# cgtuebingen/ggnn

Hardware: AMD Instinct MI355X
Metric: queries/sec @ recall@10 (SIFT1M-shaped, k=10) (higher is better)
Workload: dtype f32

## Files before the change

ggnn_amd/_lib.py:

```python
import ctypes as C
import os

_HERE = os.path.dirname(os.path.abspath(__file__))
LIB_PATH = os.path.join(_HERE, "csrc", "libggnn_amd.so")
if os.environ.get("GGNN_TEST_HOOKS") == "1" and os.environ.get("GGNN_AMD_LIB"):
    LIB_PATH = os.environ["GGNN_AMD_LIB"]

OK, INVALID_ARGUMENT, INVALID_STATE, OUT_OF_RANGE, OUT_OF_MEMORY, DEVICE_ERROR, UNSUPPORTED, \
    IO_ERROR = range(8)
F32, U8, F16, BF16 = 0, 1, 2, 3
I8 = 5
CPU, GPU = 0, 1


class GraphConfig(C.Structure):
    _fields_ = [(n, C.c_uint32) for n in
                ("N", "D", "KBuild", "KF", "G", "S", "S0", "S0_off", "SG", "SG_off", "N_all",
                 "ST_all")] + [("Bs", C.c_uint32 * 4), ("Ns", C.c_uint32 * 4),
                               ("Ns_offsets", C.c_uint32 * 4), ("STs_offsets", C.c_uint32 * 4)]

    def as_dict(self):
        d = {}
        for name, _ in self._fields_:
            v = getattr(self, name)
# ... 125 lines not shown
    "ggnn_last_build_work": (_int, [_vp, C.POINTER(BuildWork)]),
    "ggnn_last_query_parts": (_int, [_vp, C.POINTER(_u32)]),
    "ggnn_rccl_ranks": (_int, [_vp, C.POINTER(_u32)]),
    "ggnn_set_hook": (_int, [C.c_char_p, C.c_int64]),
    "ggnn_reset_hook": (_int, [C.c_char_p]),
    "ggnn_get_hook": (_int, [C.c_char_p, C.POINTER(C.c_int64)]),
    "ggnn_set_log_level": (None, [_int]),
    "ggnn_graph_config_init": (_int, [_u32, _u32, _u32, _cfgp]),
    "ggnn_query_sizing": (_int, [_u32, _u32, _u32, C.POINTER(_u32), C.POINTER(_u32)]),
    "ggnn_op_dist_layout": (_int, [_u32, _int, C.POINTER(_u32), C.POINTER(_u32)]),
    "ggnn_op_query": (_int, [_vp, _int, _u32, _u32, _vp, _u32, _vp, _u32, _vp, _u32, _vp, _u32,
                             _f32, _u32, _int, _u32, _u32, _vp, _vp, _vp, _vp, _vp]),
    "ggnn_prescreen_sizes": (_int, [_u32, _u32, _int, C.POINTER(_u32), C.POINTER(_sz),
                                    C.POINTER(_sz)]),
    "ggnn_op_prescreen_encode": (_int, [_vp, _u32, _u32, _int, _vp, _vp, _vp, _vp]),
    "ggnn_op_prescreen_probe": (_int, [_vp, _vp, _u32, _int, _vp, _u32, _vp, _u32, _vp, _vp, _vp,
                                       _vp]),
    "ggnn_op_query_prescreened": (_int, [_vp, _u32, _u32, _vp, _vp, _vp, _u32, _vp, _u32, _vp, _u32,
                                         _vp, _u32, _f32, _u32, _int, _u32, _u32, _vp, _vp, _vp,
                                         _vp, _vp, _vp]),
    "ggnn_op_query_filtered": (_int, [_vp, _int, _u32, _u32, _vp, _vp, _vp, _u32, _vp, _u32, _vp,
                                      _u32, _vp, _u32, _f32, _u32, _int, _u32, _u32, _vp, _vp, _vp,
                                      _vp, _vp, _vp, _u32, _vp]),
    "ggnn_op_bf_query_filtered": (_int, [_vp, _int, _u32, _u32, _vp, _u32, _u32, _int, _vp, _vp,
                                         _vp, _u32, _vp]),
    "ggnn_op_query_filtered_by": (_int, [_vp, _int, _u32, _u32, _vp, _vp, _vp, _u32, _vp, _u32,
                                         _vp, _u32, _vp, _u32, _f32, _u32, _int, _u32, _u32, _vp,
                                         _vp, _vp, _vp, _vp, _vp, _u32, _u64, _vp, _u32, _vp]),
    "ggnn_op_bf_query_filtered_by": (_int, [_vp, _int, _u32, _u32, _vp, _u32, _u32, _int, _vp,
                                            _vp, _vp, _u32, _u64, _vp, _u32, _vp]),
# ... 140 lines not shown
```

ggnn_amd/csrc/common.hpp:

```cpp
#pragma once
#include <hip/hip_runtime.h>

#include <cstdint>
#include <cstdio>
#include <stdexcept>
#include <string>

#include "../../include/ggnn_c.h"

namespace ggnn_amd {

constexpr int kWave = 64;
constexpr int32_t kEmptyKey = -1;
constexpr uint32_t kLayers = 4;
constexpr uint32_t kKBlock = 32;

struct Error : std::runtime_error {
  ggnn_status status;
  Error(ggnn_status s, const std::string& msg) : std::runtime_error(msg), status(s) {}
};

#define GGNN_HIP_CHECK(expr)                                                                  \
  do {                                                                                        \
    hipError_t _e = (expr);                                                                   \
// ... 121 lines not shown
  uint32_t num_start;
  const float* nn1_stats;
  uint32_t k_query;
  float tau_query;
  uint32_t max_iterations;
  ggnn_measure measure;
  uint32_t shards_per_gpu, on_gpu_shard;
  int32_t* ids;
  float* dists;
  uint32_t* n_dist;
  uint32_t* n_pop;
  const uint8_t* ps_codes{nullptr};
  const float* ps_params{nullptr};
  uint32_t ps_Dc{0};
  bool ps_lossless{false};
  uint32_t* n_rows{nullptr};
  const uint32_t* filter_bits{nullptr};
  uint32_t filter_bit_offset{0};
  FilterTable filter_table{};
  LabelSetSpec label_sets{};
  LabelRangeSpec label_ranges{};
  LabelMaskSpec label_masks{};
};
void launch_query(const QueryLaunch& a, hipStream_t stream);

constexpr int kPsHeaderFloats = 8;
inline uint32_t prescreen_code_dim(uint32_t D)
{
  if (D <= 64) {
    uint32_t p = 16;
    while (p < D)
      p <<= 1;
    return p;
  }
  return (D + 63u) / 64u * 64u;
}
size_t prescreen_param_floats(uint32_t D);
size_t prescreen_scratch_floats(uint32_t N, uint32_t D, ggnn_measure measure);
void launch_prescreen_encode(const float* base, uint32_t N, uint32_t D, ggnn_measure measure,
                             uint8_t* codes, float* params, float* scratch, hipStream_t stream);
void launch_prescreen_probe(const uint8_t* codes, const float* params, uint32_t D,
                            ggnn_measure measure, const float* query, uint32_t Nq,
                            const int32_t* cand, uint32_t M, const float* crit, int32_t* reject,
                            float* s_out, hipStream_t stream);

struct BfLaunch {
  const void* base;
  const void* query;
  ggnn_dtype dtype;
  uint32_t N_base, D, Nq, k_query;
  ggnn_measure measure;
  int32_t* ids;
  float* dists;
  uint32_t* n_rescanned{nullptr};
  const uint32_t* filter_bits{nullptr};
// ... 180 lines not shown
```

ggnn_amd/csrc/engine.hpp:

```cpp
#pragma once
#include <dlfcn.h>
#include <rccl/rccl.h>

#include <algorithm>
#include <atomic>
#include <cstdlib>
#include <cstring>
#include <filesystem>
#include <fstream>
#include <exception>
#include <memory>
#include <mutex>
#include <thread>
#include <vector>

#include "common.hpp"
#include "hooks.hpp"

namespace ggnn_amd {

struct DeviceBuffer {
  void* p{nullptr};
  size_t bytes{0};
  DeviceBuffer() = default;
// ... 93 lines not shown
    GGNN_HIP_CHECK(hipEventSynchronize(b));
    GGNN_HIP_CHECK(hipEventElapsedTime(&ms, a, b));
    return ms;
  }
};

struct Shard {
  uint32_t global_id{0};
  DeviceBuffer pool;
  int32_t* graph{nullptr};
  int32_t* translation{nullptr};
  int32_t* selection{nullptr};
  float* nn1_stats{nullptr};
  bool ready{false};
  DeviceBuffer ps_codes, ps_params;
  int ps_state{0};
  bool ps_lossless{false};
  ggnn_measure ps_measure{GGNN_EUCLIDEAN};

  static size_t pool_bytes(const ggnn_graph_config& c)
  {
    return (static_cast<size_t>(c.N_all) * c.KBuild + 2 * static_cast<size_t>(c.ST_all)) * 4 +
           2 * sizeof(float);
  }
  void view(const ggnn_graph_config& c, void* slot_pool)
  {
    graph = static_cast<int32_t*>(slot_pool);
    translation = graph + static_cast<size_t>(c.N_all) * c.KBuild;
    selection = translation + c.ST_all;
    nn1_stats = reinterpret_cast<float*>(selection + c.ST_all);
// ... 517 lines not shown
```

ggnn_amd/csrc/engine_cabi.cpp:

```cpp
#include "engine.hpp"
#include "traversal.hpp"

namespace {
thread_local std::string g_create_error;

template <typename F>
ggnn_status guarded(ggnn_t* h, F&& f)
{
  DeviceRestoreGuard restore;
  try {
    f();
    return GGNN_OK;
  }
  catch (const Error& e) {
    (h ? h->last_error : g_create_error) = e.what();
    return e.status;
  }
  catch (const std::bad_alloc&) {
    (h ? h->last_error : g_create_error) = "out of host memory";
    return GGNN_OUT_OF_MEMORY;
  }
  catch (const std::exception& e) {
    (h ? h->last_error : g_create_error) = e.what();
    return GGNN_DEVICE_ERROR;
// ... 984 lines not shown
    if (scratch_floats)
      *scratch_floats = prescreen_scratch_floats(N_base, D, measure);
  });
}

ggnn_status ggnn_op_prescreen_encode(const float* base, uint32_t N_base, uint32_t D,
                                     ggnn_measure measure, uint8_t* codes, float* params,
                                     float* scratch, void* stream)
{
  return guarded(nullptr, [&] {
    launch_prescreen_encode(base, N_base, D, measure, codes, params, scratch,
                            static_cast<hipStream_t>(stream));
  });
}

ggnn_status ggnn_op_prescreen_probe(const uint8_t* codes, const float* params, uint32_t D,
                                    ggnn_measure measure, const float* query, uint32_t Nq,
                                    const int32_t* cand, uint32_t M, const float* crit,
                                    int32_t* reject, float* s_out, void* stream)
{
  return guarded(nullptr, [&] {
    launch_prescreen_probe(codes, params, D, measure, query, Nq, cand, M, crit, reject, s_out,
                           static_cast<hipStream_t>(stream));
  });
}

ggnn_status ggnn_op_query_prescreened(const float* base, uint32_t N_base, uint32_t D,
                                      const uint8_t* codes, const float* params,
                                      const float* query, uint32_t Nq, const int32_t* graph0,
                                      uint32_t KBuild, const int32_t* start, uint32_t num_start,
// ... 666 lines not shown
```

ggnn_amd/csrc/engine_query.cpp:

```cpp
#include "engine.hpp"

void ggnn_handle::check_query(uint64_t Nq, uint32_t D, ggnn_dtype dtype, const void* q) const
{
  GGNN_REQUIRE(dtype == base_dtype, GGNN_INVALID_ARGUMENT,
               "query data type does not match base data type");
  GGNN_REQUIRE(D == base_D, GGNN_INVALID_ARGUMENT, "query dimension does not match the base");
  GGNN_REQUIRE(Nq < 0xffffffffull, GGNN_INVALID_ARGUMENT, "too many queries");
  GGNN_REQUIRE(!Nq || q != nullptr, GGNN_INVALID_ARGUMENT, "query pointer is null");
}

ggnn_handle::Staged ggnn_handle::stage_query(DeviceCtx& ctx, const void* q, uint64_t Nq, uint32_t D, ggnn_dtype dtype,
                   ggnn_location loc, int q_gpu)
{
  Staged s;
  if (!Nq)
    return s;
  const size_t es = dtype_size(dtype);
  const bool padded = pad_D != base_D;
  if (loc == GGNN_GPU && q_gpu == ctx.device && !padded &&
      (reinterpret_cast<uintptr_t>(q) & 15u) == 0) {
    s.ptr = q;
    return s;
  }
  const hipMemcpyKind kind = loc == GGNN_GPU ? hipMemcpyDefault : hipMemcpyHostToDevice;
// ... 29 lines not shown
                 r.k,
                 r.tau,
                 r.max_iterations,
                 r.measure,
                 shards_per_gpu,
                 si,
                 d_ids,
                 d_dists,
                 nullptr,
                 nullptr};
  if (use_prescreen) {
    ql.ps_codes = sh.ps_codes.as<uint8_t>();
    ql.ps_params = sh.ps_params.as<float>();
    ql.ps_Dc = prescreen_code_dim(pad_D);
    ql.ps_lossless = sh.ps_lossless;
  }
  ql.filter_bits = df.bits;
  ql.filter_bit_offset = sh.global_id * cfg.N;
  ql.filter_table = df.table;
  ql.label_sets = df.set;
  ql.label_ranges = df.ranges;
  ql.label_masks = df.masks;
  return ql;
}

void ggnn_handle::query_device(DeviceCtx& ctx, const QueryRequest& r, const void* d_query,
                               int32_t* d_ids, float* d_dists, const QueryFilter& filter)
{
  hipStream_t stream = ctx.stream;
  const uint32_t spg = shards_per_gpu;
// ... 919 lines not shown
```

ggnn_amd/csrc/engine_residency.cpp:

```cpp
#include "engine.hpp"

void ggnn_handle::pin_host_copy()
{
  if (base_host_copy_registered || base_host_copy.empty())
    return;
  if (hipHostRegister(base_host_copy.data(), base_host_copy.size(), hipHostRegisterDefault) ==
      hipSuccess)
    base_host_copy_registered = true;
  else
    (void)hipGetLastError();
}

void ggnn_handle::drop_host_copy()
{
  if (base_host_copy_registered)
    (void)hipHostUnregister(base_host_copy.data());
  base_host_copy_registered = false;
  base_host_copy.clear();
  base_host_copy.shrink_to_fit();
}

bool ggnn_handle::has_graph() const
{
  if (!prepared || devs.empty())
// ... 155 lines not shown
  if (sh.ps_state != 0 && sh.ps_measure != measure) {
    ctx.activate();
    GGNN_HIP_CHECK(hipStreamSynchronize(ctx.stream));
    for (int i = 0; i < DeviceCtx::kShardStreams; ++i)
      if (ctx.shard_stream[i])
        GGNN_HIP_CHECK(hipStreamSynchronize(ctx.shard_stream[i]));
    sh.ps_state = 0;
    sh.ps_lossless = false;
  }
  if (sh.ps_state == 0) {
    const uint32_t Dc = prescreen_code_dim(pad_D);
    DeviceBuffer scratch;
    try {
      sh.ps_codes.alloc(static_cast<size_t>(cfg.N) * Dc);
      sh.ps_params.alloc(prescreen_param_floats(pad_D) * 4);
      scratch.alloc(prescreen_scratch_floats(cfg.N, pad_D, measure) * 4);
    }
    catch (const Error& e) {
      if (e.status != GGNN_OUT_OF_MEMORY)
        throw;
      (void)hipGetLastError();
      sh.ps_codes.release();
      sh.ps_params.release();
      sh.ps_state = -1;
      sh.ps_measure = measure;
      GGNN_LOG(0, "[GPU: %d] no memory for the pre-screen copy of part %u, continuing without",
               ctx.device, sh.global_id);
      return false;
    }
    launch_prescreen_encode(static_cast<const float*>(shard_base(ctx, si)), cfg.N, pad_D, measure,
                            sh.ps_codes.as<uint8_t>(), sh.ps_params.as<float>(),
                            scratch.as<float>(), ctx.stream);
    float header[kPsHeaderFloats];
    GGNN_HIP_CHECK(hipMemcpyAsync(header, sh.ps_params.p, sizeof(header), hipMemcpyDeviceToHost,
                                  ctx.stream));
    GGNN_HIP_CHECK(hipStreamSynchronize(ctx.stream));
    sh.ps_state = header[4] != 0.f ? 1 : -1;
    sh.ps_lossless = sh.ps_state > 0 && header[5] != 0.f;
    sh.ps_measure = measure;
    GGNN_LOG(1, "[GPU: %d] pre-screen copy of part %u (%s): scale %g, max coding error %g%s",
             ctx.device, sh.global_id, measure == GGNN_EUCLIDEAN ? "L2" : "cosine", header[0],
             header[2], sh.ps_state > 0 ? "" : " (unusable, disabled)");
    if (sh.ps_state < 0) {
      sh.ps_codes.release();
      sh.ps_params.release();
    }
  }
  return sh.ps_state > 0;
}

std::filesystem::path ggnn_handle::part_file(uint32_t shard) const
{
  return graph_dir / ("part_" + std::to_string(shard) + ".ggnn");
}

void ggnn_handle::store()
{
  GGNN_REQUIRE(has_graph(), GGNN_INVALID_STATE, "There is no graph to store.");
  if (graph_dir.empty())
    graph_dir = std::filesystem::current_path();
// ... 69 lines not shown
```

ggnn_amd/csrc/prescreen.hip:

```cpp
#include "traversal.hpp"

namespace ggnn_amd {

namespace {

constexpr uint32_t kPsBlocks = 1024;
constexpr uint32_t kPsThreads = 256;

__global__ void __launch_bounds__(kPsThreads)
    ps_minmax_kernel(const float* base, uint32_t N, uint32_t D, uint32_t B, const float* inv_norm,
                     float* partial, uint32_t* flags)
{
  const uint32_t b = blockIdx.x;
  bool bad = false;
  for (uint32_t d = threadIdx.x; d < D; d += kPsThreads) {
    float mn = inf_f(), mx = -inf_f();
    for (uint64_t r = b; r < N; r += B) {
      float v = base[r * D + d];
      bad |= !(fabsf(v) < inf_f());
      if (inv_norm)
        v *= inv_norm[r];
      bad |= !(fabsf(v) < inf_f());
      mn = fminf(mn, v);
      mx = fmaxf(mx, v);
// ... 145 lines not shown
                               (static_cast<double>(o) + static_cast<double>(s) * c);
            err += res * res;
          }
        }
      }
      *reinterpret_cast<uint4*>(out + d0) = make_uint4(w[0], w[1], w[2], w[3]);
    }
  }
  for (uint32_t off = lpr / 2; off; off >>= 1)
    err += __shfl_xor(err, off);
  if (row < N && g == 0 && err > 0.0) {
    const float e = static_cast<float>(sqrt(err)) * (1.f + 1e-6f) +
                    1e-12f * (params[3] + 255.f * s * sqrtf(static_cast<float>(Dc)));
    atomicMax(reinterpret_cast<uint32_t*>(params + 2), __float_as_uint(e));
  }
}

template <int LPR, int NCH, int MODE>
__global__ void __launch_bounds__(kWave)
    ps_probe_kernel(const uint8_t* codes, const float* params, uint32_t D, uint32_t Dc,
                    const float* query, uint32_t Nq, const int32_t* cand, uint32_t M,
                    const float* crit, int32_t* reject, float* s_out)
{
  using PS = Prescreen<LPR, NCH, MODE>;
  const uint32_t n = block_linear_index();
  if (n >= Nq)
    return;
  PS ps;
  ps.load(codes, params, Dc, query + static_cast<size_t>(n) * D, D);
  const int grp = threadIdx.x / LPR;
// ... 53 lines not shown
  if (inv_norm)
    hipLaunchKernelGGL(ps_inv_norm_kernel, grid, dim3(kPsThreads), 0, stream, base, N, D, lpr,
                       inv_norm);
  hipLaunchKernelGGL(ps_minmax_kernel, dim3(B), dim3(kPsThreads), 0, stream, base, N, D, B,
                     inv_norm, scratch, flags);
  hipLaunchKernelGGL(ps_finalize_kernel, dim3(1), dim3(kPsThreads), 0, stream, scratch, flags, D,
                     Dc, B, static_cast<int>(measure), params);
  hipLaunchKernelGGL(ps_encode_kernel, grid, dim3(kPsThreads), 0, stream, base, N, D, Dc, lpr,
                     inv_norm, codes, params);
  hipLaunchKernelGGL(ps_retry_kernel, dim3(1), dim3(1), 0, stream, params, Dc);
  hipLaunchKernelGGL(ps_encode_kernel, grid, dim3(kPsThreads), 0, stream, base, N, D, Dc, lpr,
                     inv_norm, codes, params);
  GGNN_HIP_CHECK(hipGetLastError());
}

void launch_prescreen_probe(const uint8_t* codes, const float* params, uint32_t D,
                            ggnn_measure measure, const float* query, uint32_t Nq,
                            const int32_t* cand, uint32_t M, const float* crit, int32_t* reject,
                            float* s_out, hipStream_t stream)
{
  if (!Nq || !M)
    return;
  GGNN_REQUIRE(D >= 1 && D <= 4096 && D % 4 == 0, GGNN_INVALID_ARGUMENT,
               "D must be a multiple of 4 in [4, 4096]");
  const uint32_t Dc = prescreen_code_dim(D);
  const uint32_t chunks = Dc / 16;
#define GGNN_PROBE(LPR, NCH)                                                                      \
  do {                                                                                            \
    if (measure == GGNN_EUCLIDEAN)                                                                \
      hipLaunchKernelGGL((ps_probe_kernel<LPR, NCH, kL2>), grid_for(Nq), dim3(kWave), 0, stream,  \
// ... 19 lines not shown
```

ggnn_amd/csrc/query.hip:

```cpp
#include <algorithm>

#include "query_wave.hpp"

namespace ggnn_amd {

#ifndef GGNN_QUERY_WAVES
#define GGNN_QUERY_WAVES 7
#endif
#ifndef GGNN_QUERY_WAVES_GR
#define GGNN_QUERY_WAVES_GR 7
#endif

template <typename BaseT, int LPR, int NCH, int R, int MODE, class PSC, int HB = 0, bool EARLY = false,
          bool GR = false>
__global__ void __launch_bounds__(kWave) __attribute__((
    amdgpu_waves_per_eu((R == 1 && NCH <= 3) ? (GR ? GGNN_QUERY_WAVES_GR : GGNN_QUERY_WAVES) : 1)))
query_kernel(const QueryArgs a)
{
  using FILT = NoIdFilter;
#include "query_wave_body.inc"
}

template <typename BaseT, int LPR, int NCH, int MODE, class PSC>
__global__ void __launch_bounds__(kWave) query_kernel_lds(const QueryArgs a)
// ... 19 lines not shown
#endif

struct QueryLadder {
  template <typename BaseT, int LPR, int NCH, int MODE, class PSC>
  static void launch(const QueryArgs& args, hipStream_t stream)
  {
    const uint32_t sorted = args.sorted;
    const size_t lds = wave_lds_bytes(args.cache);
    const auto go = [&](void (*kernel)(QueryArgs), size_t lds_bytes) {
      launch_wave_per_query(kernel, args, lds_bytes, stream);
    };
    const bool fits = PSC::enabled || NCH == 1;
    const uint32_t hb = (sorted <= 64 && fits) ? vis_hash_regs(args.cache - sorted) : 0;
    if constexpr (early_rows_layout<LPR, NCH, PSC>()) {
      using PSX = typename ExactOf<PSC>::type;
      const bool exact = args.ps_lossless != 0 && !std::is_same<PSX, PSC>::value;
      const bool tagged = hb == 0 && fits && args.ring && (args.tag_bits == 8 || args.tag_bits == 9);
      const bool tagged_ringless = tagged && args.max_iters <= args.cache - sorted &&
                                   hook(kHookQueryGlobalRing) != 0;
      if (args.KBuild <= 8 * kEarlySteps && sorted <= 64 && tagged_ringless &&
          hook(kHookQueryEarly) != 0) {
        const size_t tag_lds = tag_set_lds_bytes(sorted, args.cache - sorted) +
                               DistEngine<BaseT, LPR, NCH, PSC::enabled>::kQueryLdsBytes;
        if (args.tag_bits == 8)
          go(exact ? query_kernel<BaseT, LPR, NCH, 1, MODE, PSX, -8, true, true>
                   : query_kernel<BaseT, LPR, NCH, 1, MODE, PSC, -8, true, true>, tag_lds);
        else
          go(exact ? query_kernel<BaseT, LPR, NCH, 1, MODE, PSX, -9, true, true>
                   : query_kernel<BaseT, LPR, NCH, 1, MODE, PSC, -9, true, true>, tag_lds);
        return;
      }
// ... 103 lines not shown
        throw;
      (void)hipGetLastError();
      args.ring = nullptr;
    }
  }
  ScratchGuard ring_guard{args.ring, stream};
  if (use_ps) {
    GGNN_REQUIRE(a.ps_Dc == prescreen_code_dim(a.D), GGNN_INVALID_ARGUMENT,
                 "pre-screen code rows must have prescreen_code_dim(D) bytes");
    GGNN_REQUIRE((reinterpret_cast<uintptr_t>(a.ps_codes) & 15u) == 0 &&
                     (reinterpret_cast<uintptr_t>(a.ps_params) & 15u) == 0,
                 GGNN_INVALID_ARGUMENT, "pre-screen buffers must be 16-byte aligned");
    args.ps_codes = a.ps_codes;
    args.ps_params = a.ps_params;
    args.ps_Dc = a.ps_Dc;
    args.ps_lossless = (a.ps_lossless && a.measure == GGNN_EUCLIDEAN && hook(kHookPsExact) != 0) ? 1u : 0u;
  }

  if (a.label_masks.labels) {
    GGNN_REQUIRE(!a.label_sets.labels && !a.label_ranges.labels, GGNN_INVALID_ARGUMENT,
                 "label masks cannot be combined with label sets or label ranges in one launch");
    args.filter_bits = a.filter_bits;
    args.filter_bit_offset = a.filter_bit_offset;
    launch_query_labelmask(args, a.filter_table, a.label_masks, use_ps, a.measure, a.dtype, stream);
  }
  else if (a.label_ranges.labels) {
    GGNN_REQUIRE(!a.label_sets.labels, GGNN_INVALID_ARGUMENT,
                 "label ranges and label sets cannot be combined in one launch");
    args.filter_bits = a.filter_bits;
    args.filter_bit_offset = a.filter_bit_offset;
    launch_query_labelrange(args, a.filter_table, a.label_ranges, use_ps, a.measure, a.dtype, stream);
// ... 69 lines not shown
```

ggnn_amd/csrc/query_args.hpp:

```cpp
#pragma once
#include "common.hpp"

namespace ggnn_amd {

struct QueryArgs {
  const void* base;
  const void* query;
  const int32_t* graph0;
  const int32_t* start;
  const float* nn1_stats;
  int32_t* ids;
  float* dists;
  uint32_t* n_dist;
  uint32_t* n_pop;
  uint2* n_rows;
  uint32_t D, Nq, N_base, KBuild, num_start, KQuery, sorted, cache, max_iters;
  uint32_t shards_per_gpu, on_gpu_shard;
  float tau;
  const uint8_t* ps_codes;
  const float* ps_params;
  uint32_t ps_Dc;
  uint32_t vis_slots;
  int32_t* ring;
  uint32_t tag_bits;
  const uint32_t* filter_bits;
  uint32_t filter_bit_offset;
  uint32_t ps_lossless;
};

struct FilteredQueryArgs : QueryArgs {
  FilterTable filter_table;
};

struct LabelSetQueryArgs : FilteredQueryArgs {
  LabelSetSpec set;
};

struct LabelRangeQueryArgs : FilteredQueryArgs {
  LabelRangeSpec range;
};

struct LabelMaskQueryArgs : FilteredQueryArgs {
  LabelMaskSpec mask;
// ... 4 lines not shown
```

ggnn_amd/csrc/query_filtered.hip:

```cpp
#include <algorithm>

#include "query_wave.hpp"

namespace ggnn_amd {

template <int NCH, int MODE, class PSC, bool EARLY>
constexpr int filtered_waves()
{
  return (EARLY && PSC::enabled && (NCH == 2 || MODE == kCos)) ? 6 : 7;
}

template <typename BaseT, int LPR, int NCH, int R, int MODE, class PSC, int HB = 0, bool EARLY = false>
__global__ void __launch_bounds__(kWave) __attribute__((
    amdgpu_waves_per_eu((R == 1 && NCH <= 3) ? filtered_waves<NCH, MODE, PSC, EARLY>() : 1)))
query_filtered_kernel(const FilteredQueryArgs a)
{
  static_assert(HB >= 0, "the filtered kernels keep their visited ring in LDS");
  using FILT = IdFilter;
  constexpr bool GR = false;
#include "query_wave_body.inc"
}

template <typename BaseT, int LPR, int NCH, int MODE, class PSC>
__global__ void __launch_bounds__(kWave) query_filtered_kernel_lds(const FilteredQueryArgs a)
// ... 127 lines not shown

template <class FILT>
struct FilteredLadder {
  template <typename BaseT, int LPR, int NCH, int MODE, class PSC, class ARGS>
  static void launch(const ARGS& args, hipStream_t stream)
  {
    const uint32_t sorted = args.sorted;
    if constexpr (early_rows_layout<LPR, NCH, PSC>()) {
      const uint32_t hb = sorted <= 64 ? vis_hash_regs(args.cache - sorted) : 0;
      if (hb != 0 && args.KBuild <= 8 * kEarlySteps && hook(kHookQueryEarly) != 0) {
        const size_t qrow = DistEngine<BaseT, LPR, NCH, PSC::enabled>::kQueryLdsBytes;
        using PSX = std::conditional_t<std::is_same<FILT, LabelSetFilter>::value ||
                                           std::is_same<FILT, LabelRangeFilter>::value ||
                                           std::is_same<FILT, LabelMaskFilter>::value,
                                       PSC, typename ExactOf<PSC>::type>;
        const bool exact = args.ps_lossless != 0 && !std::is_same<PSX, PSC>::value;
        if (hb == 1)
          launch_wave_per_query(exact ? filtered_kernel<FILT, BaseT, LPR, NCH, 1, MODE, PSX, 1, true>()
                                      : filtered_kernel<FILT, BaseT, LPR, NCH, 1, MODE, PSC, 1, true>(),
                                args, wave_lds_bytes(args.cache, 1) + qrow, stream);
        else
          launch_wave_per_query(exact ? filtered_kernel<FILT, BaseT, LPR, NCH, 1, MODE, PSX, 2, true>()
                                      : filtered_kernel<FILT, BaseT, LPR, NCH, 1, MODE, PSC, 2, true>(),
                                args, wave_lds_bytes(args.cache, 2) + qrow, stream);
        return;
      }
    }
    launch_query_ladder<PSC>(sorted, [&](auto regs) {
      constexpr int R = decltype(regs)::value;
      if constexpr (R == 0)
        launch_query_lds_list(filtered_kernel_lds<FILT, BaseT, LPR, NCH, MODE, PSC>(), args, stream);
// ... 208 lines not shown
```

ggnn_amd/csrc/query_wave.hpp:

```cpp
#pragma once
#include "traversal.hpp"
#include "query_args.hpp"

namespace ggnn_amd {

template <class PSC, typename BaseT>
GGNN_DEV void load_prescreen(PSC& ps, const QueryArgs& a, const BaseT* qrow)
{
  if constexpr (PSC::enabled)
    ps.template load<PsExact<PSC>::value>(a.ps_codes, a.ps_params, a.ps_Dc,
                                          reinterpret_cast<const float*>(qrow), a.D);
}

template <class FILT, class ARGS>
GGNN_DEV FILT wave_filter(const ARGS& a, const uint32_t n)
{
  if constexpr (std::is_same<FILT, LabelMaskFilter>::value)
    return LabelMaskFilter(a.filter_bits, a.filter_bit_offset, a.filter_table, a.mask, n);
  else if constexpr (std::is_same<FILT, LabelRangeFilter>::value)
    return LabelRangeFilter(a.filter_bits, a.filter_bit_offset, a.filter_table, a.range, n);
  else if constexpr (std::is_same<FILT, LabelSetFilter>::value)
    return LabelSetFilter(a.filter_bits, a.filter_bit_offset, a.filter_table, a.set, n);
  else if constexpr (std::is_same<FILT, LabelFilter>::value)
    return LabelFilter(a.filter_bits, a.filter_bit_offset, a.filter_table, n);
// ... 24 lines not shown
    return false;
  if (std::is_same_v<FILT, IdFilter> && sizeof(BaseT) == 2 && !PSC::enabled && LPR == 16 && NCH == 4 &&
      MODE == kCos && HB == 0)
    return false;
  if (FILT::enabled || NCH != 2)
    return true;
  if (std::is_same_v<BaseT, float> && PSC::enabled && EARLY && !GR) {
    if (LPR == 16)
      return HB != 2;
    if (LPR == 8)
      return MODE == kL2 ? !(HB == 1 || HB == 2) : !(HB == 0 || HB == 1);
  }
  if (is_byte_row<BaseT> && !PSC::enabled && !EARLY && !GR && LPR == 8 && MODE == kCos)
    return !is_tag_set(HB);
  return true;
}


template <int LPR, int NCH, class PSC>
constexpr bool early_rows_layout()
{
  return PSC::enabled ? (PsLayout<PSC>::lpr == 8 && PsLayout<PSC>::nch == 1) : (LPR == 8 && NCH == 1);
}

template <class ARGS>
void launch_wave_per_query(void (*kernel)(ARGS), const ARGS& args, size_t lds_bytes, hipStream_t stream)
{
  hipLaunchKernelGGL(kernel, grid_for(args.Nq), dim3(kWave), lds_bytes, stream, args);
}

// ... 80 lines not shown
```

ggnn_amd/csrc/query_wave_body.inc:

```
  extern __shared__ __attribute__((aligned(16))) int lds_raw[];
  const WaveLds lds(lds_raw, (is_tag_set(HB) || GR) ? a.sorted : a.cache);
  const int lane = threadIdx.x;
  const uint32_t n = block_linear_index();
  if (n >= a.Nq)
    return;

  const BaseT* base = static_cast<const BaseT*>(a.base);
  const BaseT* query = static_cast<const BaseT*>(a.query);

  const float nn1 = a.nn1_stats[1];
  const float xi = (MODE == kL2) ? (nn1 * nn1) * a.tau * a.tau : nn1 * a.tau;

  using DE = DistEngine<BaseT, LPR, NCH, EARLY && PSC::enabled>;
  DE de;
  de.template load_query<MODE>(
      base, a.D, query + static_cast<size_t>(n) * a.D,
      lds_raw + (is_tag_set(HB) ? tag_set_lds_ints(a.sorted, static_cast<uint32_t>(-HB))
                                : wave_lds_ints(GR ? a.sorted : a.cache, HB)));
  PSC ps;
  constexpr bool kExactCodes = PsExact<PSC>::value;
  static_assert(!kExactCodes || EARLY, "exact distances from codes: early-rows kernels only");
  load_prescreen(ps, a, query + static_cast<size_t>(n) * a.D);

  SortedList<R, HB, GR, query_select_push<BaseT, LPR, NCH, R, MODE, PSC, HB, EARLY, GR, FILT>()> sl;
// ... 40 lines not shown
            (static_cast<uint64_t>(static_cast<uint32_t>(uni(static_cast<int>(rp >> 32)))) << 32) |
            static_cast<uint32_t>(uni(static_cast<int>(rp))));
        cand = in_row ? row[lane] : kEmptyKey;
      }
      else
        cand = in_row ? a.graph0[static_cast<size_t>(static_cast<uint32_t>(anchor)) * a.KBuild + lane]
                      : kEmptyKey;
      auto prefetch_head_row = [&]() {
        spec_key = sl.key_at(sl.BEST);
        spec_row = a.graph0[static_cast<size_t>(static_cast<uint32_t>(max(spec_key, 0))) * a.KBuild +
                            min(lane, static_cast<int>(a.KBuild) - 1)];
        __builtin_amdgcn_s_setprio(1);
      };
      request_filter_words(idf, cand);
      if constexpr (PSC::enabled) {
        EarlyRows<PSC> er;
        er.issue(ps, cand);
        __builtin_amdgcn_s_setprio(0);
        sl.pop_commit(anchor, lds.known);
        cnt_dist += fetch_early<MODE, true, kExactCodes>(sl, de, lds, cand, er, ps, cnt_rows,
                                                  prefetch_head_row, nullptr, idf);
      }
      else {
        EarlyRows<DE> er;
        er.issue(de, cand);
        __builtin_amdgcn_s_setprio(0);
        sl.pop_commit(anchor, lds.known);
        cnt_dist += fetch_early<MODE>(sl, de, lds, cand, er, ps, cnt_rows, prefetch_head_row,
                                      nullptr, idf);
      }
      continue;
// ... 49 lines not shown
```

ggnn_amd/csrc/traversal.hpp:

```cpp
#pragma once
#include <cstdlib>
#include <type_traits>

#include "common.hpp"
#include "hooks.hpp"

namespace ggnn_amd {

#define GGNN_DEV __device__ __forceinline__

#ifdef GGNN_PHASE_CYCLES
static __device__ unsigned long long g_phase_acc[16];
GGNN_DEV void phase_tick(int i)
{
  extern __shared__ __attribute__((aligned(16))) int ph_lds[];
  unsigned long long* p = reinterpret_cast<unsigned long long*>(ph_lds + 4096);
  asm volatile("s_waitcnt vmcnt(0) lgkmcnt(0)" ::: "memory");
  const unsigned long long t = __builtin_amdgcn_s_memtime();
  if (threadIdx.x == 0) {
    if (i >= 0)
      p[1 + i] += t - p[0];
    p[0] = t;
  }
}
// ... 85 lines not shown
  v += dpp_f<0x4E>(v);
  if (LPR >= 8)
    v += dpp_f<0x141>(v);
  if (LPR >= 16)
    v += dpp_f<0x140>(v);
  if (LPR >= 32) {
    const auto r = __builtin_amdgcn_permlane16_swap(__float_as_uint(v), __float_as_uint(v), false,
                                                    false);
    v = __uint_as_float(r[0]) + __uint_as_float(r[1]);
  }
  if (LPR >= 64) {
    const auto r = __builtin_amdgcn_permlane32_swap(__float_as_uint(v), __float_as_uint(v), false,
                                                    false);
    v = __uint_as_float(r[0]) + __uint_as_float(r[1]);
  }
  return v;
}

struct WaveLds {
  int* known;
  int* ckeys;
  float* cd0;
  float* cd1;
  GGNN_DEV WaveLds(int* base, int cache)
      : known(base), ckeys(base + cache), cd0(reinterpret_cast<float*>(base + cache + 32)),
        cd1(reinterpret_cast<float*>(base + cache + 64))
  {
  }
  static constexpr size_t extra_ints = 96;
};
// ... 1188 lines not shown
  {
    uint32_t ab = 0, bb = qq;
#pragma unroll
    for (int c = 0; c < NCH; ++c) {
      ab = __builtin_amdgcn_udot4(v[c].x, qc[c].x, ab, false);
      ab = __builtin_amdgcn_udot4(v[c].y, qc[c].y, ab, false);
      ab = __builtin_amdgcn_udot4(v[c].z, qc[c].z, ab, false);
      ab = __builtin_amdgcn_udot4(v[c].w, qc[c].w, ab, false);
      bb = __builtin_amdgcn_udot4(v[c].x, v[c].x, bb, false);
      bb = __builtin_amdgcn_udot4(v[c].y, v[c].y, bb, false);
      bb = __builtin_amdgcn_udot4(v[c].z, v[c].z, bb, false);
      bb = __builtin_amdgcn_udot4(v[c].w, v[c].w, bb, false);
    }
    return static_cast<float>(bb - 2u * ab);
  }

  GGNN_DEV float threshold(float crit) const
  {
    if (!(crit < inf_f()) || !usable)
      return inf_f();
    if (MODE_ == kCos)
      crit = 2.f * (crit + m) * (1.f + m);
    float t = __builtin_amdgcn_sqrtf(crit) * (1.f + m) + slack;
    t = t * inv_s * (1.f + m);
    return t * t * (1.f + m);
  }
};

template <int LPR_, int NCH_, int MODE_ = kL2>
struct PrescreenExact : Prescreen<LPR_, NCH_, MODE_> {
};
template <class PS>
struct PsExact {
  static constexpr bool value = false;
};
template <int LPR, int NCH, int MODE>
struct PsExact<PrescreenExact<LPR, NCH, MODE>> {
  static constexpr bool value = true;
};
template <class PS>
struct ExactOf {
  using type = PS;
};
template <>
struct ExactOf<Prescreen<8, 1, kL2>> {
// ... 428 lines not shown
    const int k = rdlane(ck, j);
    replay_push(sl, k, d);
  }
  GGNN_TICK(8);
  return nsurv;
}
template <int MODE, bool FILTER, class SL, class DE>
GGNN_DEV int fetch(SL& sl, const DE& de, const WaveLds& lds, int cand,
                   const int32_t* translation)
{
  uint2 rows = make_uint2(0u, 0u);
  return fetch<MODE, FILTER>(sl, de, lds, cand, translation, NoPrescreen{}, rows);
}

constexpr int kEarlySteps = 3;
template <class RD>
struct EarlyRows {
  static_assert(RD::LPR == 8 && RD::NCH == 1, "early rows: 8 lanes x one 16-byte chunk per row");
  int kk[kEarlySteps];
  typename RD::Chunk v[kEarlySteps][1];
  GGNN_DEV void issue(const RD& rd, const int cand, const int32_t* translation = nullptr)
  {
    const int grp = threadIdx.x >> 3;
#pragma unroll
    for (int s = 0; s < kEarlySteps; ++s)
      kk[s] = __builtin_amdgcn_ds_bpermute((grp * kEarlySteps + s) << 2, cand);
    int m[kEarlySteps];
#pragma unroll
    for (int s = 0; s < kEarlySteps; ++s) {
      m[s] = max(kk[s], 0);
      if (translation)
        m[s] = translation[m[s]];
    }
// ... 9 lines not shown
          v[s][0] = rd.load_chunk(rd.row_ptr(m[s]), 0);
        else
          v[s][0] = typename RD::Chunk{};
      }
      asm volatile("");
    }
  }
  template <typename T>
  static GGNN_DEV T of_my_step(const T x0, const T x1, const T x2)
  {
    const int w = threadIdx.x & 7;
    T r = x2;
    r = (w == 1) ? x1 : r;
    r = (w == 0) ? x0 : r;
    return r;
  }
};

template <class SL>
GGNN_DEV void replay_lanes(SL& sl, unsigned long long m, const int k_of, const float d_of)
{
  while (m) {
    const int j = __ffsll(static_cast<long long>(m)) - 1;
    m &= m - 1;
    const float d = rdlanef(d_of, j);
    const int k = rdlane(k_of, j);
    replay_push(sl, k, d);
  }
}

// ... 6 lines not shown
  constexpr bool kFiltered = std::remove_reference_t<FILT>::enabled;
  const int lane = threadIdx.x;
  const int grp = lane >> 3, w = lane & 7;
  cand = sl.template filter<false, COUNT>(lower_half_to_both(cand), lds.known);
  const unsigned surv = static_cast<unsigned>(__ballot(lane < 32 && cand != kEmptyKey));
  const int nsurv = __popc(surv);
  after_filter();
  const bool alive = w < kEarlySteps && ((surv >> (grp * kEarlySteps + w)) & 1u);
  if constexpr (PS::enabled) {
    if (nsurv == 0)
      return 0;
    constexpr bool kExact = EXACT && MODE == kL2;
    if constexpr (kExact) {
      static_assert(PS::LPR == 8 && PS::NCH == 1, "lossless codes: sums of at most 128 dimensions");
      static_assert(PS::LPR * PS::NCH * 16 * 255 * 255 < (1 << 24), "s^2 * S must be exact");
    }
    bool exact = false;
    if constexpr (kExact)
      exact = ps.s2 != 0.f;
    const float crit = sl.criteria();
    const float s_thr = exact ? crit : ps.threshold(crit);
    if (s_thr < inf_f())
      rows.y += nsurv;
    float S[kEarlySteps];
#pragma unroll
    for (int s = 0; s < kEarlySteps; ++s)
      S[s] = group_sum<8>(ps.partial(er.v[s]));
    const float smine = ER::of_my_step(S[0], S[1], S[2]);
    int mykey = kEmptyKey;
    if constexpr (kExact)
      mykey = ER::of_my_step(er.kk[0], er.kk[1], er.kk[2]);
    float d_of;
    int k_of;
    unsigned long long m;
    if (exact) {
      d_of = ps.s2 * smine;
      k_of = mykey;
      m = __ballot(alive && d_of < crit);
      if constexpr (!COUNT)
        m = sl.drop_sorted(m, mykey);
    }
    else {
      bool pass = alive && !(smine >= s_thr);
      unsigned long long pm = __ballot(pass);
      if constexpr (!kExact)
        mykey = ER::of_my_step(er.kk[0], er.kk[1], er.kk[2]);
// ... 162 lines not shown
```

ggnn_amd/ops.py:

```python
import ctypes as C

import torch

from . import _lib
from ._lib import GraphConfig, check, lib

EUCLIDEAN, COSINE = 0, 1


_DTYPE_CODES = {torch.float32: _lib.F32, torch.uint8: _lib.U8, torch.float16: _lib.F16,
                torch.bfloat16: _lib.BF16, torch.int8: _lib.I8}


def _dtype_code(t):
    code = _DTYPE_CODES.get(t.dtype)
    if code is None:
        raise TypeError("base/query must be int8, float32, uint8, float16 or bfloat16")
    return code


def _ptr(t):
    return None if t is None else t.data_ptr()


# ... 48 lines not shown
    import ctypes as C
    dc, pf, sf = C.c_uint32(), C.c_size_t(), C.c_size_t()
    check(lib().ggnn_prescreen_sizes(N, D, measure, C.byref(dc), C.byref(pf), C.byref(sf)))
    return dc.value, pf.value, sf.value


def prescreen_encode(base, measure=EUCLIDEAN):
    _need(base, torch.float32, "base")
    dc, pf, sf = prescreen_sizes(base.shape[0], base.shape[1], measure)
    codes = torch.empty((base.shape[0], dc), dtype=torch.uint8, device=base.device)
    params = torch.empty(pf, dtype=torch.float32, device=base.device)
    scratch = torch.empty(sf, dtype=torch.float32, device=base.device)
    check(lib().ggnn_op_prescreen_encode(_ptr(base), base.shape[0], base.shape[1], measure,
                                         _ptr(codes), _ptr(params), _ptr(scratch), _stream()))
    return codes, params


def prescreen_probe(codes, params, query, cand, crit, measure=EUCLIDEAN):
    _need(codes, torch.uint8, "codes"), _need(params, torch.float32, "params")
    _need(query, torch.float32, "query"), _need(cand, torch.int32, "cand")
    _need(crit, torch.float32, "crit")
    Nq, M = cand.shape
    reject = torch.empty((Nq, M), dtype=torch.int32, device=codes.device)
    s_out = torch.empty((Nq, M), dtype=torch.float32, device=codes.device)
    check(lib().ggnn_op_prescreen_probe(_ptr(codes), _ptr(params), query.shape[1], measure,
                                        _ptr(query), Nq, _ptr(cand), M, _ptr(crit), _ptr(reject),
                                        _ptr(s_out), _stream()))
    return reject, s_out


# ... 762 lines not shown
```

include/ggnn_c.h:

```cpp
#ifndef GGNN_C_H
#define GGNN_C_H

#include <stddef.h>
#include <stdint.h>

#ifdef __cplusplus
extern "C" {
#endif

typedef enum {
  GGNN_OK = 0,
  GGNN_INVALID_ARGUMENT = 1,
  GGNN_INVALID_STATE = 2,
  GGNN_OUT_OF_RANGE = 3,
  GGNN_OUT_OF_MEMORY = 4,
  GGNN_DEVICE_ERROR = 5,
  GGNN_UNSUPPORTED = 6,
  GGNN_IO_ERROR = 7
} ggnn_status;

typedef enum { GGNN_EUCLIDEAN = 0, GGNN_COSINE = 1 } ggnn_measure;
typedef enum { GGNN_F32 = 0, GGNN_U8 = 1, GGNN_F16 = 2, GGNN_BF16 = 3, GGNN_I8 = 5 } ggnn_dtype;
typedef enum { GGNN_CPU = 0, GGNN_GPU = 1 } ggnn_location;

// ... 260 lines not shown
                                uint32_t* chunks_per_lane);

ggnn_status ggnn_op_query(const void* base, ggnn_dtype dtype, uint32_t N_base, uint32_t D,
                          const void* query, uint32_t Nq, const int32_t* graph0,
                          uint32_t KBuild, const int32_t* start, uint32_t num_start,
                          const float* nn1_stats, uint32_t k_query, float tau_query,
                          uint32_t max_iterations, ggnn_measure measure,
                          uint32_t shards_per_gpu, uint32_t on_gpu_shard, int32_t* ids,
                          float* dists, uint32_t* n_dist, uint32_t* n_pop, void* stream);

ggnn_status ggnn_prescreen_sizes(uint32_t N_base, uint32_t D, ggnn_measure measure,
                                 uint32_t* code_dim, size_t* param_floats, size_t* scratch_floats);
ggnn_status ggnn_op_prescreen_encode(const float* base, uint32_t N_base, uint32_t D,
                                     ggnn_measure measure, uint8_t* codes, float* params,
                                     float* scratch, void* stream);
ggnn_status ggnn_op_prescreen_probe(const uint8_t* codes, const float* params, uint32_t D,
                                    ggnn_measure measure, const float* query, uint32_t Nq,
                                    const int32_t* cand, uint32_t M, const float* crit,
                                    int32_t* reject, float* s_out, void* stream);
ggnn_status ggnn_op_query_prescreened(const float* base, uint32_t N_base, uint32_t D,
                                      const uint8_t* codes, const float* params,
                                      const float* query, uint32_t Nq, const int32_t* graph0,
                                      uint32_t KBuild, const int32_t* start, uint32_t num_start,
                                      const float* nn1_stats, uint32_t k_query, float tau_query,
                                      uint32_t max_iterations, ggnn_measure measure,
                                      uint32_t shards_per_gpu, uint32_t on_gpu_shard, int32_t* ids,
                                      float* dists, uint32_t* n_dist, uint32_t* n_pop,
                                      uint32_t* n_rows, void* stream);

ggnn_status ggnn_op_query_filtered(const void* base, ggnn_dtype dtype, uint32_t N_base, uint32_t D,
// ... 264 lines not shown
```

Before: 12.13 million.

## Precompute code-row squared norms for exact prescreen distances via dot products

Adds a kernel that computes the squared norm of every uint8 prescreen code row when the index is built, and stores it per shard. In the lossless Euclidean prescreen path, the early-rows stage then computes distances as |q|^2 + |c|^2 - 2<q,c>, using udot4 dot products plus one gathered norm per candidate, instead of summing squared differences. This trades a 4-byte norm load per candidate and extra memory for cheaper arithmetic in the traversal's inner loop. The query argument struct is repacked to carry the norms pointer in place of the lossless flag while keeping its layout.

Result: slower. 9.118 million (-24.8%).

```diff
diff --git a/ggnn_amd/_lib.py b/ggnn_amd/_lib.py
--- a/ggnn_amd/_lib.py
+++ b/ggnn_amd/_lib.py
@@ -163,6 +163,7 @@
     "ggnn_prescreen_sizes": (_int, [_u32, _u32, _int, C.POINTER(_u32), C.POINTER(_sz),
                                     C.POINTER(_sz)]),
     "ggnn_op_prescreen_encode": (_int, [_vp, _u32, _u32, _int, _vp, _vp, _vp, _vp]),
+    "ggnn_op_prescreen_norms": (_int, [_vp, _u32, _u32, _vp, _vp]),
     "ggnn_op_prescreen_probe": (_int, [_vp, _vp, _u32, _int, _vp, _u32, _vp, _u32, _vp, _vp, _vp,
                                        _vp]),
     "ggnn_op_query_prescreened": (_int, [_vp, _u32, _u32, _vp, _vp, _vp, _u32, _vp, _u32, _vp, _u32,
diff --git a/ggnn_amd/csrc/common.hpp b/ggnn_amd/csrc/common.hpp
--- a/ggnn_amd/csrc/common.hpp
+++ b/ggnn_amd/csrc/common.hpp
@@ -159,6 +159,7 @@
   const float* ps_params{nullptr};
   uint32_t ps_Dc{0};
   bool ps_lossless{false};
+  const uint32_t* ps_norms{nullptr};
   uint32_t* n_rows{nullptr};
   const uint32_t* filter_bits{nullptr};
   uint32_t filter_bit_offset{0};
@@ -184,6 +185,8 @@
 size_t prescreen_scratch_floats(uint32_t N, uint32_t D, ggnn_measure measure);
 void launch_prescreen_encode(const float* base, uint32_t N, uint32_t D, ggnn_measure measure,
                              uint8_t* codes, float* params, float* scratch, hipStream_t stream);
+void launch_prescreen_norms(const uint8_t* codes, uint32_t N, uint32_t Dc, uint32_t* norms,
+                            hipStream_t stream);
 void launch_prescreen_probe(const uint8_t* codes, const float* params, uint32_t D,
                             ggnn_measure measure, const float* query, uint32_t Nq,
                             const int32_t* cand, uint32_t M, const float* crit, int32_t* reject,
diff --git a/ggnn_amd/csrc/engine.hpp b/ggnn_amd/csrc/engine.hpp
--- a/ggnn_amd/csrc/engine.hpp
+++ b/ggnn_amd/csrc/engine.hpp
@@ -131,6 +131,7 @@
   float* nn1_stats{nullptr};
   bool ready{false};
   DeviceBuffer ps_codes, ps_params;
+  DeviceBuffer ps_norms;
   int ps_state{0};
   bool ps_lossless{false};
   ggnn_measure ps_measure{GGNN_EUCLIDEAN};
diff --git a/ggnn_amd/csrc/engine_cabi.cpp b/ggnn_amd/csrc/engine_cabi.cpp
--- a/ggnn_amd/csrc/engine_cabi.cpp
+++ b/ggnn_amd/csrc/engine_cabi.cpp
@@ -1022,6 +1022,14 @@
   });
 }
 
+ggnn_status ggnn_op_prescreen_norms(const uint8_t* codes, uint32_t N_base, uint32_t code_dim,
+                                    uint32_t* norms, void* stream)
+{
+  return guarded(nullptr, [&] {
+    launch_prescreen_norms(codes, N_base, code_dim, norms, static_cast<hipStream_t>(stream));
+  });
+}
+
 ggnn_status ggnn_op_prescreen_probe(const uint8_t* codes, const float* params, uint32_t D,
                                     ggnn_measure measure, const float* query, uint32_t Nq,
                                     const int32_t* cand, uint32_t M, const float* crit,
diff --git a/ggnn_amd/csrc/engine_query.cpp b/ggnn_amd/csrc/engine_query.cpp
--- a/ggnn_amd/csrc/engine_query.cpp
+++ b/ggnn_amd/csrc/engine_query.cpp
@@ -67,6 +67,7 @@
     ql.ps_params = sh.ps_params.as<float>();
     ql.ps_Dc = prescreen_code_dim(pad_D);
     ql.ps_lossless = sh.ps_lossless;
+    ql.ps_norms = sh.ps_norms.as<uint32_t>();
   }
   ql.filter_bits = df.bits;
   ql.filter_bit_offset = sh.global_id * cfg.N;
diff --git a/ggnn_amd/csrc/engine_residency.cpp b/ggnn_amd/csrc/engine_residency.cpp
--- a/ggnn_amd/csrc/engine_residency.cpp
+++ b/ggnn_amd/csrc/engine_residency.cpp
@@ -193,6 +193,7 @@
     try {
       sh.ps_codes.alloc(static_cast<size_t>(cfg.N) * Dc);
       sh.ps_params.alloc(prescreen_param_floats(pad_D) * 4);
+      sh.ps_norms.alloc(static_cast<size_t>(cfg.N) * sizeof(uint32_t));
       scratch.alloc(prescreen_scratch_floats(cfg.N, pad_D, measure) * 4);
     }
     catch (const Error& e) {
@@ -201,6 +202,7 @@
       (void)hipGetLastError();
       sh.ps_codes.release();
       sh.ps_params.release();
+      sh.ps_norms.release();
       sh.ps_state = -1;
       sh.ps_measure = measure;
       GGNN_LOG(0, "[GPU: %d] no memory for the pre-screen copy of part %u, continuing without",
@@ -210,6 +212,8 @@
     launch_prescreen_encode(static_cast<const float*>(shard_base(ctx, si)), cfg.N, pad_D, measure,
                             sh.ps_codes.as<uint8_t>(), sh.ps_params.as<float>(),
                             scratch.as<float>(), ctx.stream);
+    launch_prescreen_norms(sh.ps_codes.as<uint8_t>(), cfg.N, Dc, sh.ps_norms.as<uint32_t>(),
+                           ctx.stream);
     float header[kPsHeaderFloats];
     GGNN_HIP_CHECK(hipMemcpyAsync(header, sh.ps_params.p, sizeof(header), hipMemcpyDeviceToHost,
                                   ctx.stream));
@@ -223,6 +227,7 @@
     if (sh.ps_state < 0) {
       sh.ps_codes.release();
       sh.ps_params.release();
+      sh.ps_norms.release();
     }
   }
   return sh.ps_state > 0;
diff --git a/ggnn_amd/csrc/prescreen.hip b/ggnn_amd/csrc/prescreen.hip
--- a/ggnn_amd/csrc/prescreen.hip
+++ b/ggnn_amd/csrc/prescreen.hip
@@ -183,6 +183,29 @@
                     1e-12f * (params[3] + 255.f * s * sqrtf(static_cast<float>(Dc)));
     atomicMax(reinterpret_cast<uint32_t*>(params + 2), __float_as_uint(e));
   }
+}
+
+__global__ void __launch_bounds__(kPsThreads)
+    ps_norms_kernel(const uint8_t* codes, uint32_t N, uint32_t Dc, uint32_t* norms)
+{
+  constexpr uint32_t kLpr = 8;
+  const uint64_t row = static_cast<uint64_t>(block_linear_index()) * (kPsThreads / kLpr) +
+                       threadIdx.x / kLpr;
+  const uint32_t g = threadIdx.x % kLpr;
+  uint32_t acc = 0;
+  if (row < N) {
+    const uint8_t* c = codes + row * Dc;
+    for (uint32_t d0 = g * 16; d0 < Dc; d0 += kLpr * 16) {
+      const uint4 v = *reinterpret_cast<const uint4*>(c + d0);
+      acc = __builtin_amdgcn_udot4(v.x, v.x, acc, false);
+      acc = __builtin_amdgcn_udot4(v.y, v.y, acc, false);
+      acc = __builtin_amdgcn_udot4(v.z, v.z, acc, false);
+      acc = __builtin_amdgcn_udot4(v.w, v.w, acc, false);
+    }
+  }
+  acc = group_sum_u32<kLpr>(acc);
+  if (row < N && g == 0)
+    norms[row] = acc;
 }
 
 template <int LPR, int NCH, int MODE>
@@ -266,6 +289,22 @@
   GGNN_HIP_CHECK(hipGetLastError());
 }
 
+void launch_prescreen_norms(const uint8_t* codes, uint32_t N, uint32_t Dc, uint32_t* norms,
+                            hipStream_t stream)
+{
+  if (!N)
+    return;
+  GGNN_REQUIRE(Dc >= 16 && Dc <= 4096 && Dc % 16 == 0, GGNN_INVALID_ARGUMENT,
+               "code rows must have a multiple of 16 bytes in [16, 4096]");
+  GGNN_REQUIRE((reinterpret_cast<uintptr_t>(codes) & 15u) == 0 &&
+                   (reinterpret_cast<uintptr_t>(norms) & 3u) == 0,
+               GGNN_INVALID_ARGUMENT, "code rows must be 16-byte aligned");
+  const uint32_t rows_per_block = kPsThreads / 8;
+  const dim3 grid = grid_for((static_cast<uint64_t>(N) + rows_per_block - 1) / rows_per_block);
+  hipLaunchKernelGGL(ps_norms_kernel, grid, dim3(kPsThreads), 0, stream, codes, N, Dc, norms);
+  GGNN_HIP_CHECK(hipGetLastError());
+}
+
 void launch_prescreen_probe(const uint8_t* codes, const float* params, uint32_t D,
                             ggnn_measure measure, const float* query, uint32_t Nq,
                             const int32_t* cand, uint32_t M, const float* crit, int32_t* reject,
diff --git a/ggnn_amd/csrc/query.hip b/ggnn_amd/csrc/query.hip
--- a/ggnn_amd/csrc/query.hip
+++ b/ggnn_amd/csrc/query.hip
@@ -57,7 +57,7 @@
     const uint32_t hb = (sorted <= 64 && fits) ? vis_hash_regs(args.cache - sorted) : 0;
     if constexpr (early_rows_layout<LPR, NCH, PSC>()) {
       using PSX = typename ExactOf<PSC>::type;
-      const bool exact = args.ps_lossless != 0 && !std::is_same<PSX, PSC>::value;
+      const bool exact = args.exact_codes() && !std::is_same<PSX, PSC>::value;
       const bool tagged = hb == 0 && fits && args.ring && (args.tag_bits == 8 || args.tag_bits == 9);
       const bool tagged_ringless = tagged && args.max_iters <= args.cache - sorted &&
                                    hook(kHookQueryGlobalRing) != 0;
@@ -191,7 +191,8 @@
     args.ps_codes = a.ps_codes;
     args.ps_params = a.ps_params;
     args.ps_Dc = a.ps_Dc;
-    args.ps_lossless = (a.ps_lossless && a.measure == GGNN_EUCLIDEAN && hook(kHookPsExact) != 0) ? 1u : 0u;
+    if (a.ps_lossless && a.ps_norms && a.measure == GGNN_EUCLIDEAN && hook(kHookPsExact) != 0)
+      args.set_ps_norms(a.ps_norms);
   }
 
   if (a.label_masks.labels) {
diff --git a/ggnn_amd/csrc/query_args.hpp b/ggnn_amd/csrc/query_args.hpp
--- a/ggnn_amd/csrc/query_args.hpp
+++ b/ggnn_amd/csrc/query_args.hpp
@@ -23,10 +23,25 @@
   uint32_t vis_slots;
   int32_t* ring;
   uint32_t tag_bits;
+  uint32_t ps_norms_lo;
   const uint32_t* filter_bits;
   uint32_t filter_bit_offset;
-  uint32_t ps_lossless;
+  uint32_t ps_norms_hi;
+
+  __host__ __device__ uint64_t ps_norms() const
+  {
+    return (static_cast<uint64_t>(ps_norms_hi) << 32) | ps_norms_lo;
+  }
+  void set_ps_norms(const uint32_t* p)
+  {
+    ps_norms_lo = static_cast<uint32_t>(reinterpret_cast<uint64_t>(p));
+    ps_norms_hi = static_cast<uint32_t>(reinterpret_cast<uint64_t>(p) >> 32);
+  }
+  bool exact_codes() const { return (ps_norms_lo | ps_norms_hi) != 0; }
 };
+static_assert(sizeof(QueryArgs) == 184 && offsetof(QueryArgs, ps_norms_lo) == 164 &&
+                  offsetof(QueryArgs, filter_bits) == 168 && offsetof(QueryArgs, ps_norms_hi) == 180,
+              "the argument block of the query kernels keeps its layout");
 
 struct FilteredQueryArgs : QueryArgs {
   FilterTable filter_table;
diff --git a/ggnn_amd/csrc/query_filtered.hip b/ggnn_amd/csrc/query_filtered.hip
--- a/ggnn_amd/csrc/query_filtered.hip
+++ b/ggnn_amd/csrc/query_filtered.hip
@@ -165,7 +165,7 @@
                                            std::is_same<FILT, LabelRangeFilter>::value ||
                                            std::is_same<FILT, LabelMaskFilter>::value,
                                        PSC, typename ExactOf<PSC>::type>;
-        const bool exact = args.ps_lossless != 0 && !std::is_same<PSX, PSC>::value;
+        const bool exact = args.exact_codes() && !std::is_same<PSX, PSC>::value;
         if (hb == 1)
           launch_wave_per_query(exact ? filtered_kernel<FILT, BaseT, LPR, NCH, 1, MODE, PSX, 1, true>()
                                       : filtered_kernel<FILT, BaseT, LPR, NCH, 1, MODE, PSC, 1, true>(),
diff --git a/ggnn_amd/csrc/query_wave.hpp b/ggnn_amd/csrc/query_wave.hpp
--- a/ggnn_amd/csrc/query_wave.hpp
+++ b/ggnn_amd/csrc/query_wave.hpp
@@ -7,7 +7,10 @@
 template <class PSC, typename BaseT>
 GGNN_DEV void load_prescreen(PSC& ps, const QueryArgs& a, const BaseT* qrow)
 {
-  if constexpr (PSC::enabled)
+  if constexpr (PsExact<PSC>::value)
+    ps.load_exact(a.ps_codes, a.ps_params, a.ps_Dc, a.ps_norms(),
+                  reinterpret_cast<const float*>(qrow), a.D);
+  else if constexpr (PSC::enabled)
     ps.template load<PsExact<PSC>::value>(a.ps_codes, a.ps_params, a.ps_Dc,
                                           reinterpret_cast<const float*>(qrow), a.D);
 }
@@ -62,6 +65,15 @@
   if (is_byte_row<BaseT> && !PSC::enabled && !EARLY && !GR && LPR == 8 && MODE == kCos)
     return !is_tag_set(HB);
   return true;
+}
+
+template <typename BaseT, int LPR, int NCH, int R, int MODE, class PSC, int HB, bool EARLY, bool GR,
+          class FILT>
+constexpr bool query_code_norms()
+{
+  if (!PsExact<PSC>::value)
+    return false;
+  return !(FILT::enabled && NCH == 2 && HB == 2);
 }
 
 
diff --git a/ggnn_amd/csrc/query_wave_body.inc b/ggnn_amd/csrc/query_wave_body.inc
--- a/ggnn_amd/csrc/query_wave_body.inc
+++ b/ggnn_amd/csrc/query_wave_body.inc
@@ -78,7 +78,7 @@
       };
       request_filter_words(idf, cand);
       if constexpr (PSC::enabled) {
-        EarlyRows<PSC> er;
+        EarlyRows<PSC, query_code_norms<BaseT, LPR, NCH, R, MODE, PSC, HB, EARLY, GR, FILT>()> er;
         er.issue(ps, cand);
         __builtin_amdgcn_s_setprio(0);
         sl.pop_commit(anchor, lds.known);
diff --git a/ggnn_amd/csrc/traversal.hpp b/ggnn_amd/csrc/traversal.hpp
--- a/ggnn_amd/csrc/traversal.hpp
+++ b/ggnn_amd/csrc/traversal.hpp
@@ -123,6 +123,18 @@
                                                     false);
     v = __uint_as_float(r[0]) + __uint_as_float(r[1]);
   }
+  return v;
+}
+template <int LPR>
+GGNN_DEV uint32_t group_sum_u32(uint32_t v)
+{
+  static_assert(LPR <= 16, "integer group sum: one DPP row");
+  v += static_cast<uint32_t>(__builtin_amdgcn_update_dpp(0, static_cast<int>(v), 0xB1, 0xf, 0xf, true));
+  v += static_cast<uint32_t>(__builtin_amdgcn_update_dpp(0, static_cast<int>(v), 0x4E, 0xf, 0xf, true));
+  if (LPR >= 8)
+    v += static_cast<uint32_t>(__builtin_amdgcn_update_dpp(0, static_cast<int>(v), 0x141, 0xf, 0xf, true));
+  if (LPR >= 16)
+    v += static_cast<uint32_t>(__builtin_amdgcn_update_dpp(0, static_cast<int>(v), 0x140, 0xf, 0xf, true));
   return v;
 }
 
@@ -1341,6 +1353,18 @@
     }
     return static_cast<float>(bb - 2u * ab);
   }
+  GGNN_DEV uint32_t dot(const uint4 (&v)[NCH]) const
+  {
+    uint32_t ab = 0;
+#pragma unroll
+    for (int c = 0; c < NCH; ++c) {
+      ab = __builtin_amdgcn_udot4(v[c].x, qc[c].x, ab, false);
+      ab = __builtin_amdgcn_udot4(v[c].y, qc[c].y, ab, false);
+      ab = __builtin_amdgcn_udot4(v[c].z, qc[c].z, ab, false);
+      ab = __builtin_amdgcn_udot4(v[c].w, qc[c].w, ab, false);
+    }
+    return ab;
+  }
 
   GGNN_DEV float threshold(float crit) const
   {
@@ -1356,6 +1380,16 @@
 
 template <int LPR_, int NCH_, int MODE_ = kL2>
 struct PrescreenExact : Prescreen<LPR_, NCH_, MODE_> {
+  using Norms = const __attribute__((address_space(1))) uint32_t*;
+  Norms norms;
+  uint32_t QQ;
+  GGNN_DEV void load_exact(const uint8_t* codes_, const float* params, uint32_t Dc_,
+                           const uint64_t norms_, const float* qrow, uint32_t D)
+  {
+    this->template load<true>(codes_, params, Dc_, qrow, D);
+    norms = reinterpret_cast<Norms>(norms_);
+    QQ = static_cast<uint32_t>(uni(static_cast<int>(group_sum_u32<LPR_>(this->qq))));
+  }
 };
 template <class PS>
 struct PsExact {
@@ -1814,9 +1848,11 @@
 }
 
 constexpr int kEarlySteps = 3;
-template <class RD>
+template <class RD, bool NORMS = false>
 struct EarlyRows {
   static_assert(RD::LPR == 8 && RD::NCH == 1, "early rows: 8 lanes x one 16-byte chunk per row");
+  static_assert(!NORMS, "code-row norms: kernels of PrescreenExact<8, 1, kL2>");
+  static constexpr bool kNorms = false;
   int kk[kEarlySteps];
   typename RD::Chunk v[kEarlySteps][1];
   GGNN_DEV void issue(const RD& rd, const int cand, const int32_t* translation = nullptr)
@@ -1856,6 +1892,48 @@
     r = (w == 1) ? x1 : r;
     r = (w == 0) ? x0 : r;
     return r;
+  }
+};
+template <>
+struct EarlyRows<PrescreenExact<8, 1, kL2>, true> {
+  using RD = PrescreenExact<8, 1, kL2>;
+  static constexpr bool kNorms = true;
+  int mykey;
+  uint32_t norm;
+  typename RD::Chunk v[kEarlySteps][1];
+  GGNN_DEV void issue(const RD& rd, const int cand)
+  {
+    const int grp = threadIdx.x >> 3;
+    int kk[kEarlySteps];
+#pragma unroll
+    for (int s = 0; s < kEarlySteps; ++s)
+      kk[s] = __builtin_amdgcn_ds_bpermute((grp * kEarlySteps + s) << 2, cand);
+    mykey = of_my_step(kk[0], kk[1], kk[2]);
+    int m[kEarlySteps];
+#pragma unroll
+    for (int s = 0; s < kEarlySteps; ++s)
+      m[s] = max(kk[s], 0);
+    if (rd.all_chunks) {
+#pragma unroll
+      for (int s = 0; s < kEarlySteps; ++s)
+        v[s][0] = rd.load_chunk(rd.row_ptr(m[s]), 0);
+    }
+    else {
+#pragma unroll
+      for (int s = 0; s < kEarlySteps; ++s) {
+        if (rd.chunk_valid(0))
+          v[s][0] = rd.load_chunk(rd.row_ptr(m[s]), 0);
+        else
+          v[s][0] = typename RD::Chunk{};
+      }
+      asm volatile("");
+    }
+    norm = rd.norms[static_cast<uint32_t>(max(mykey, 0))];
+  }
+  template <typename T>
+  static GGNN_DEV T of_my_step(const T x0, const T x1, const T x2)
+  {
+    return EarlyRows<Prescreen<8, 1, kL2>>::of_my_step(x0, x1, x2);
   }
 };
 
@@ -1892,6 +1970,8 @@
     if constexpr (kExact) {
       static_assert(PS::LPR == 8 && PS::NCH == 1, "lossless codes: sums of at most 128 dimensions");
       static_assert(PS::LPR * PS::NCH * 16 * 255 * 255 < (1 << 24), "s^2 * S must be exact");
+      static_assert(2 * PS::LPR * PS::NCH * 16 * 255 * 255 < (1 << 24),
+                    "|cq|^2 + |c|^2 must be exact too (code-row norms)");
     }
     bool exact = false;
     if constexpr (kExact)
@@ -1900,14 +1980,26 @@
     const float s_thr = exact ? crit : ps.threshold(crit);
     if (s_thr < inf_f())
       rows.y += nsurv;
-    float S[kEarlySteps];
-#pragma unroll
-    for (int s = 0; s < kEarlySteps; ++s)
-      S[s] = group_sum<8>(ps.partial(er.v[s]));
-    const float smine = ER::of_my_step(S[0], S[1], S[2]);
+    float smine;
     int mykey = kEmptyKey;
-    if constexpr (kExact)
-      mykey = ER::of_my_step(er.kk[0], er.kk[1], er.kk[2]);
+    if constexpr (kExact && ER::kNorms) {
+      uint32_t ab[kEarlySteps];
+#pragma unroll
+      for (int s = 0; s < kEarlySteps; ++s)
+        ab[s] = group_sum_u32<8>(ps.dot(er.v[s]));
+      const uint32_t abmine = ER::of_my_step(ab[0], ab[1], ab[2]);
+      smine = static_cast<float>(ps.QQ + er.norm - 2u * abmine);
+      mykey = er.mykey;
+    }
+    else {
+      float S[kEarlySteps];
+#pragma unroll
+      for (int s = 0; s < kEarlySteps; ++s)
+        S[s] = group_sum<8>(ps.partial(er.v[s]));
+      smine = ER::of_my_step(S[0], S[1], S[2]);
+      if constexpr (kExact)
+        mykey = ER::of_my_step(er.kk[0], er.kk[1], er.kk[2]);
+    }
     float d_of;
     int k_of;
     unsigned long long m;
diff --git a/ggnn_amd/ops.py b/ggnn_amd/ops.py
--- a/ggnn_amd/ops.py
+++ b/ggnn_amd/ops.py
@@ -86,6 +86,14 @@
     check(lib().ggnn_op_prescreen_encode(_ptr(base), base.shape[0], base.shape[1], measure,
                                          _ptr(codes), _ptr(params), _ptr(scratch), _stream()))
     return codes, params
+
+
+def prescreen_code_norms(codes):
+    _need(codes, torch.uint8, "codes")
+    norms = torch.empty(codes.shape[0], dtype=torch.int32, device=codes.device)
+    check(lib().ggnn_op_prescreen_norms(_ptr(codes), codes.shape[0], codes.shape[1], _ptr(norms),
+                                        _stream()))
+    return norms
 
 
 def prescreen_probe(codes, params, query, cand, crit, measure=EUCLIDEAN):
diff --git a/include/ggnn_c.h b/include/ggnn_c.h
--- a/include/ggnn_c.h
+++ b/include/ggnn_c.h
@@ -298,6 +298,8 @@
 ggnn_status ggnn_op_prescreen_encode(const float* base, uint32_t N_base, uint32_t D,
                                      ggnn_measure measure, uint8_t* codes, float* params,
                                      float* scratch, void* stream);
+ggnn_status ggnn_op_prescreen_norms(const uint8_t* codes, uint32_t N_base, uint32_t code_dim,
+                                    uint32_t* norms, void* stream);
 ggnn_status ggnn_op_prescreen_probe(const uint8_t* codes, const float* params, uint32_t D,
                                     ggnn_measure measure, const float* query, uint32_t Nq,
                                     const int32_t* cand, uint32_t M, const float* crit,
```
